# better62/MM-VQA-Healthcare

Measured on AMD Instinct MI355X. Metric: image-question pairs/sec, M3AE-base fine-tune step (fwd+bwd+AdamW) @384px, higher is better.
Workload: dtype bf16

## Files before the change

### include/m3ae_hip.h

```cpp
#ifndef M3AE_HIP_H
#define M3AE_HIP_H

#include <stdint.h>

#ifdef __cplusplus
extern "C" {
#endif

#define M3AE_ABI_VERSION 4

enum { M3AE_F32 = 0, M3AE_BF16 = 1 };
enum { M3AE_ACT_NONE = 0, M3AE_ACT_GELU = 1, M3AE_ACT_QUICKGELU = 2, M3AE_ACT_TANH = 3, M3AE_ACT_RELU = 4,
       M3AE_ACT_MULAUX = 5  };
enum { M3AE_ERR_ARG = -1, M3AE_ERR_UNSUPPORTED = -2, M3AE_ERR_ALIGN = -3, M3AE_ERR_WORKSPACE = -4 };

int m3ae_abi_version(void);
void m3ae_desc_sizes(int64_t out3[3]);
const char* m3ae_last_gemm_path(void);

typedef struct {
    int64_t M, N, K;
    int64_t batch1, batch2;
    const void* A; int64_t a_sm, a_sk, a_sb1, a_sb2;
    const void* B; int64_t b_sk, b_sn, b_sb1, b_sb2;
    void* C;       int64_t c_sm, c_sn, c_sb1, c_sb2;
    int32_t dtype_a, dtype_b, dtype_c;
    float alpha;
    int32_t accumulate;
    const float* bias;
    int32_t act;
    void* preact;
    const void* residual;
    const void* dact_aux;
    int32_t dact;
    int32_t force_generic;
    float* a_rowsum;
    float dropout_p;
    uint64_t dropout_seed;
    int32_t preact_grad;
    int32_t launch_flags;
    const void* dropout_salt;
} m3ae_gemm_desc;
enum { M3AE_GEMM_NO_PERSISTENT = 1,
       M3AE_GEMM_F32_X3 = 2,
       M3AE_GEMM_DETERMINISTIC = 4,
       M3AE_GEMM_B_TILED = 8    };
#define M3AE_GEMM_NT_VARIANT(v) ((((v) + 1) & 0xf) << 8)
#define M3AE_GEMM_TN_VARIANT(v) ((((v) + 1) & 0xf) << 12)
#define M3AE_GEMM_COL_GROUP(g) (((g) & 0xf) << 16)
int m3ae_gemm(const m3ae_gemm_desc* d, void* stream);
int m3ae_gemm_rows(const m3ae_gemm_desc* d, int64_t row_base, int64_t row_step, void* stream);
int64_t m3ae_gemm_det_workspace_bytes(const m3ae_gemm_desc* d);
int m3ae_gemm_det(const m3ae_gemm_desc* d, void* workspace, int64_t workspace_bytes, void* stream);

typedef struct {
    int64_t B, H, Lq, Lk, Dh;
    const void* q; int64_t q_sb, q_sl;
    const void* k; int64_t k_sb, k_sl;
    const void* v; int64_t v_sb, v_sl;
    void* o;       int64_t o_sb, o_sl;
    const float* key_mask;
    const float* pos_bias;
    float scale;
    int32_t causal;
    float* lse; int64_t lse_stride;
    int32_t dtype;
    void* workspace; int64_t workspace_bytes;
    const void* d_o;
    void* dq; void* dk; void* dv;
    float* delta;
    float* d_pos_bias;
    float dropout_p;
    uint64_t dropout_seed;
    const void* dropout_salt;
    int32_t launch_flags;
} m3ae_attn_desc;
enum { M3AE_ATTN_LEGACY_KERNELS = 1,
       M3AE_ATTN_F32_X3 = 2    };
int64_t m3ae_attn_workspace_bytes(const m3ae_attn_desc* d, int backward);
int m3ae_attn_fwd(const m3ae_attn_desc* d, void* stream);
int m3ae_attn_bwd(const m3ae_attn_desc* d, void* stream);
int m3ae_attn_fwd_rows(const m3ae_attn_desc* d, int64_t row_base, int64_t row_step, void* stream);
int m3ae_attn_bwd_rows(const m3ae_attn_desc* d, int64_t row_base, int64_t row_step, void* stream);
int m3ae_attn_probs(const m3ae_attn_desc* d, float* probs, int64_t p_sb, int64_t p_sh, int64_t p_sq, void* stream);
#define M3AE_ATTN_COLMEAN_F32_CHUNK 4
int64_t m3ae_attn_colmean_workspace_bytes(const m3ae_attn_desc* d);
// ... 205 lines not shown
```

### mm-vqa-healthcare_amd/csrc/gemm_mfma.hip

```cpp
#include "gemm_nt_common.h"
#include "pp_ring.h"
#include "launch.h"
#include <stdlib.h>

namespace {

constexpr int BM = 128, BN = 128, BK = 64;
constexpr int STAGE_BYTES = (BM + BN) * BK * 2;
constexpr int LDS_BYTES = 2 * STAGE_BYTES;

using namespace m3g;

template <int BM_, int BN_, int BKT, int NST, int WM, int EPI>
__global__ __launch_bounds__((BM_ / WM) * (BN_ / 64) * 64, 2) void gemm_nt_bf16_kernel(MfmaArgs a) {
    if (a.has_drop) drop_resolve(a.drop);
    constexpr int WAVES_N = BN_ / 64, NWAVES = (BM_ / WM) * WAVES_N, MI = WM / 16;
    constexpr int A_BYTES = BM_ * BKT * 2, ST_BYTES = (BM_ + BN_) * BKT * 2;
    constexpr int A_SEGS = A_BYTES / 1024 / NWAVES, B_SEGS = BN_ * BKT * 2 / 1024 / NWAVES;
    constexpr int G = A_SEGS + B_SEGS;
    extern __shared__ __attribute__((aligned(16))) char smem[];
    const int tid = threadIdx.x;
    const int lane = tid & 63;
    const int wave = __builtin_amdgcn_readfirstlane(tid >> 6);
    const int wr = wave / WAVES_N, wc = wave % WAVES_N;
// ... 554 lines not shown
        float* P = (float*)a.C + ((int64_t)split * tiles + tile_id) * (256 * 256) + ((int64_t)wave * 8 * 4 * 64 + lane) * 4;
#pragma unroll
        for (int i = 0; i < 8; ++i)
#pragma unroll
            for (int j = 0; j < 4; ++j) *(f32x4*)(P + (i * 4 + j) * 256) = acc[i][j];
        return;
    }
    if (do_rowsum && (lane & 15) == 0) {
#pragma unroll
        for (int i = 0; i < 8; ++i)
#pragma unroll
            for (int r = 0; r < 4; ++r) atomicAdd(a.a_rowsum + m0 + wr * 128 + i * 16 + 4 * (lane >> 4) + r, rsum[i][r]);
    }
    float* C = (float*)a.C;
    const bool atomic = a.splits > 1;
#pragma unroll
    for (int i = 0; i < 8; ++i)
#pragma unroll
        for (int j = 0; j < 4; ++j)
#pragma unroll
            for (int r = 0; r < 4; ++r) {
                const int64_t n1 = m0 + wr * 128 + i * 16 + 4 * (lane >> 4) + r;
                const int64_t n2 = n0 + wc * 64 + j * 16 + (lane & 15);
                float* p = C + n1 * a.ldc + n2;
                const float x = acc[i][j][r] * a.alpha;
#ifdef M3AE_EXP_TN_NOATOMIC
                asm volatile("" ::"v"(x), "v"(p));
#else
                if (atomic) atomicAdd(p, x);
                else if (a.accumulate) *p += x;
                else *p = x;
#endif
            }
}

__global__ __launch_bounds__(256) void tn_det_fold_kernel(const float* __restrict__ part, const float* __restrict__ rs_part,
                                                          float* __restrict__ C, float* __restrict__ rowsum, int64_t ldc,
                                                          int64_t M, int64_t N, int splits, int bm, int wm, float alpha,
                                                          int accumulate) {
    const int64_t plane = M * N, quads = plane / 4;
    const int waves_n = bm / 64, mi = wm / 16;
    const int64_t tile_quads = (int64_t)bm * bm / 4, tiles_n = N / bm;
    const int64_t stride = (int64_t)gridDim.x * blockDim.x;
    for (int64_t e = (int64_t)blockIdx.x * blockDim.x + threadIdx.x; e < quads; e += stride) {
        f32x4 v = *(const f32x4*)(part + e * 4);
#pragma unroll 4
        for (int sp = 1; sp < splits; ++sp) {
            const f32x4 p = *(const f32x4*)(part + sp * plane + e * 4);
            v[0] += p[0]; v[1] += p[1]; v[2] += p[2]; v[3] += p[3];
        }
        const int64_t tile = e / tile_quads;
        const int w = (int)(e - tile * tile_quads);
        const int lane = w & 63, j = (w >> 6) & 3, i = (w >> 8) % mi, wave = (w >> 8) / mi;
        const int64_t n1 = (tile / tiles_n) * bm + (wave / waves_n) * wm + i * 16 + 4 * (lane >> 4);
        const int64_t n2 = (tile % tiles_n) * bm + (wave % waves_n) * 64 + j * 16 + (lane & 15);
#pragma unroll
        for (int r = 0; r < 4; ++r) {
            float* p = C + (n1 + r) * ldc + n2;
            *p = accumulate ? *p + v[r] * alpha : v[r] * alpha;
        }
    }
    if (rowsum) {
        for (int64_t m = (int64_t)blockIdx.x * blockDim.x + threadIdx.x; m < M; m += stride) {
            float t = rs_part[m];
            for (int sp = 1; sp < splits; ++sp) t += rs_part[sp * M + m];
            rowsum[m] += t;
// ... 147 lines not shown
        g_last_path = "f32x3";
        return m3ae_gemm_f32x3(d, s, rows);
    case ROUTE_NT:
        return launch_nt(d, s, rows);
    case ROUTE_TN:
        g_last_path = "mfma_tn";
        return launch_tn(d, s);
    default:
        g_last_path = "generic";
        return m3ae_gemm_generic(d, s, rows);
    }
}

extern "C" int64_t m3ae_gemm_det_workspace_bytes(const m3ae_gemm_desc* dp) {
    if (!dp) return M3AE_ERR_ARG;
    const m3ae_gemm_desc& d = *dp;
    if (gemm_route(d) != ROUTE_TN) return 0;
    int64_t k_chunk = 0;
    const int k = tn_kernel_choice(d);
    const int64_t splits = k == 5 ? tn_pp_splits(d, &k_chunk) : tn_t_splits(d, tn_t_lds(2, k == 2 ? 32 : 64), &k_chunk);
    return tn_det_bytes(d, splits);
}

extern "C" int m3ae_gemm_det(const m3ae_gemm_desc* dp, void* workspace, int64_t workspace_bytes, void* stream) {
    if (!dp || !dp->A || !dp->B || !dp->C) return M3AE_ERR_ARG;
    const m3ae_gemm_desc& d = *dp;
    if (!(d.launch_flags & M3AE_GEMM_DETERMINISTIC)) return M3AE_ERR_ARG;
    if (d.launch_flags & M3AE_GEMM_B_TILED) return M3AE_ERR_UNSUPPORTED;
    if (gemm_route(d) != ROUTE_TN) return M3AE_ERR_UNSUPPORTED;
    if (!workspace || !aligned16(workspace) || workspace_bytes < m3ae_gemm_det_workspace_bytes(dp)) return M3AE_ERR_WORKSPACE;
    g_last_path = "mfma_tn";
    return launch_tn(d, (hipStream_t)stream, (float*)workspace);
}
```

### mm-vqa-healthcare_amd/m3ae_amd/_lib.py

```python
import ctypes as C
import os

_PKG = os.path.dirname(os.path.abspath(__file__))
DIAGNOSTIC = os.environ.get("M3AE_DIAGNOSTIC_LIB", "") == "1"
LIB_PATH = os.path.join(_PKG, "lib_diag" if DIAGNOSTIC else "lib", "libm3ae_hip.so")

F32, BF16 = 0, 1
ACT_NONE, ACT_GELU, ACT_QUICKGELU, ACT_TANH, ACT_RELU, ACT_MULAUX = 0, 1, 2, 3, 4, 5

vp, i64, i32, f32 = C.c_void_p, C.c_int64, C.c_int32, C.c_float


class GemmDesc(C.Structure):
    _fields_ = [
        ("M", i64), ("N", i64), ("K", i64), ("batch1", i64), ("batch2", i64),
        ("A", vp), ("a_sm", i64), ("a_sk", i64), ("a_sb1", i64), ("a_sb2", i64),
        ("B", vp), ("b_sk", i64), ("b_sn", i64), ("b_sb1", i64), ("b_sb2", i64),
        ("C", vp), ("c_sm", i64), ("c_sn", i64), ("c_sb1", i64), ("c_sb2", i64),
        ("dtype_a", i32), ("dtype_b", i32), ("dtype_c", i32),
        ("alpha", f32), ("accumulate", i32), ("bias", vp), ("act", i32), ("preact", vp), ("residual", vp),
        ("dact_aux", vp), ("dact", i32), ("force_generic", i32), ("a_rowsum", vp),
        ("dropout_p", f32), ("dropout_seed", C.c_uint64), ("preact_grad", i32), ("launch_flags", i32), ("dropout_salt", vp),
    ]

# ... 96 lines not shown
    "m3ae_image_resample_u8": (C.c_int, [vp, i64, vp, vp, i64, i64, i64, vp, i64, vp, vp, C.POINTER(C.c_float), C.POINTER(C.c_float), vp]),
    "m3ae_image_resample_tables": (C.c_int, [vp, i64, i64, vp, i64, vp]),
    "m3ae_image_randaug_workspace_bytes": (i64, [i64]),
    "m3ae_image_randaug_u8": (C.c_int, [vp, vp, i64, vp, i64, vp, i64, C.c_int, vp]),
    "m3ae_gemm_rows": (C.c_int, [C.POINTER(GemmDesc), i64, i64, vp]),
    "m3ae_attn_fwd_rows": (C.c_int, [C.POINTER(AttnDesc), i64, i64, vp]),
    "m3ae_attn_bwd_rows": (C.c_int, [C.POINTER(AttnDesc), i64, i64, vp]),
    "m3ae_layernorm_bwd_drop_rows": (C.c_int, [vp, vp, vp, vp, vp, vp, vp, vp, f32, C.c_uint64, vp, vp, vp, vp, i64, i64, C.c_int, i64, i64, vp]),
    "m3ae_dropout_rows": (C.c_int, [vp, vp, vp, i64, i64, f32, C.c_uint64, vp, C.c_int, i64, i64, vp]),
    "m3ae_beam_topk_workspace_bytes": (i64, [i64, i64, i64, i64]),
    "m3ae_beam_topk": (C.c_int, [vp, i64, vp, i64, i64, i64, i64, vp, i64, vp, vp, vp]),
    "m3ae_beam_step": (C.c_int, [vp, vp, vp, vp, vp, vp, vp, vp, vp, vp, vp, vp, vp, vp, i64, i64, i64, i64, i64, i64, i64, C.c_double, vp]),
    "m3ae_beam_finalize": (C.c_int, [vp, vp, vp, vp, vp, vp, vp, vp, vp, i64, i64, i64, i64, i64, i64, C.c_double, vp]),
    "m3ae_greedy_workspace_bytes": (i64, [i64, i64, i64]),
    "m3ae_greedy_argmax": (C.c_int, [vp, i64, i64, i64, i64, C.c_int, vp, i64, vp, vp]),
    "m3ae_greedy_step": (C.c_int, [vp, i64, vp, vp, vp, vp, vp, vp, i64, i64, i64, i64, i64, i64, i64, vp]),
    "m3ae_expand_samples": (C.c_int, [vp, vp, vp, i64, i64, i64, C.c_int, vp]),
    "m3ae_segment_sum_rows": (C.c_int, [vp, vp, vp, vp, i64, i64, i64, C.c_int, vp]),
    "m3ae_sumsq_workspace_bytes": (i64, [i64]),
    "m3ae_sumsq_segments": (C.c_int, [vp, i64, vp, i64, vp, i64, vp, vp, i64, vp]),
    "m3ae_clip_finalize": (C.c_int, [vp, i64, f32, f32, vp, vp]),
    "m3ae_adamw_clip": (C.c_int, [vp, vp, vp, vp, vp, i64, f32, f32, f32, f32, f32, i64, f32, vp, vp, vp]),
    "m3ae_adam": (C.c_int, [vp, vp, vp, vp, vp, i64, f32, C.c_double, C.c_double, f32, f32, i64, f32, vp]),
    "m3ae_adam_clip": (C.c_int, [vp, vp, vp, vp, vp, i64, f32, C.c_double, C.c_double, f32, f32, i64, f32, vp, vp]),
    "m3ae_sgd": (C.c_int, [vp, vp, vp, vp, i64, f32, f32, f32, f32, vp]),
    "m3ae_sgd_clip": (C.c_int, [vp, vp, vp, vp, i64, f32, f32, f32, f32, vp, vp]),
    "m3ae_layernorm_fwd_mixed": (C.c_int, [vp, vp, vp, vp, vp, vp, i64, i64, f32, vp]),
    "m3ae_layernorm_bwd_mixed": (C.c_int, [vp, vp, vp, vp, vp, vp, vp, vp, vp, vp, vp, i64, i64, vp]),
    "m3ae_layernorm_bwd_mixed_det": (C.c_int, [vp, vp, vp, vp, vp, vp, vp, vp, vp, vp, vp, i64, i64, vp]),
    "m3ae_attn_colmean_workspace_bytes": (i64, [C.POINTER(AttnDesc)]),
    "m3ae_attn_colmean": (C.c_int, [C.POINTER(AttnDesc), vp, i64, vp, i64, vp]),
    "m3ae_xattn_probs_colmean": (C.c_int, [C.POINTER(XattnDesc), C.c_int, vp, i64, vp]),
    "m3ae_heatmap_upsample": (C.c_int, [vp, i64, i64, vp, i64, i64, vp]),
}

EXPORTS = tuple(_SIGS)
_lib = None


class M3AEHipError(RuntimeError):
    pass


def lib():
    global _lib
    if _lib is None:
        if not os.path.exists(LIB_PATH):
            raise M3AEHipError(f"{LIB_PATH} is missing: build it with `python -m m3ae_amd.build` "
                               f"(or __graft_entry__.build()); this package has no CPU fallback")
        import torch
        if DIAGNOSTIC:
            import warnings
            warnings.warn(f"m3ae_amd: loading the DIAGNOSTIC library {LIB_PATH} (timing-only builds may compute wrong results)")
        l = C.CDLL(LIB_PATH)
        for name, (res, args) in _SIGS.items():
            fn = getattr(l, name)
            fn.restype, fn.argtypes = res, args
        if l.m3ae_abi_version() != ABI_VERSION:
            raise M3AEHipError(f"ABI version mismatch: library {l.m3ae_abi_version()}, binding {ABI_VERSION}")
        sizes = (i64 * 3)()
        l.m3ae_desc_sizes(sizes)
        mine = (C.sizeof(GemmDesc), C.sizeof(AttnDesc), C.sizeof(XattnDesc))
        if tuple(sizes) != mine:
            raise M3AEHipError(f"descriptor layout mismatch: library {tuple(sizes)}, binding {mine}")
        _lib = l
    return _lib
# ... 8 lines not shown
```

### mm-vqa-healthcare_amd/m3ae_amd/build.py

```python
import concurrent.futures as cf
import os
import subprocess
import sys

PKG = os.path.dirname(os.path.abspath(__file__))
ROOT = os.path.dirname(os.path.dirname(PKG))
CSRC = os.path.join(os.path.dirname(PKG), "csrc")
INC = os.path.join(ROOT, "include")
EXTRA = os.environ.get("M3AE_EXTRA_HIPCC_FLAGS", "").split()
OUT_DIR = os.path.join(PKG, "lib_diag" if EXTRA else "lib")
LIB = os.path.join(OUT_DIR, "libm3ae_hip.so")
STAMP = os.path.join(OUT_DIR, ".build_flags")
HIPCC = os.environ.get("HIPCC", "/opt/rocm/bin/hipcc")
FLAGS = ["--offload-arch=gfx950", "-O3", "-std=c++17", "-fPIC", "-Wno-unused-result", "-Wno-unused-value",
         f"-I{INC}", f"-I{CSRC}"] + EXTRA


ASM_LOAD_SOURCES = {"gemm_nt_pp2.hip": r"gemm_nt_pp2_kernel", "gemm_mfma.hip": r"gemm_nt_(bf16|pp)_kernel"}
REMARK = "-Rpass-analysis=kernel-resource-usage"


def check_no_scratch(src_name, hipcc_output):
    import re
    pat = re.compile(ASM_LOAD_SOURCES[src_name])
    name, seen, bad = None, 0, []
    for line in hipcc_output.splitlines():
        m = re.search(r"remark: Function Name: (\S+)", line)
        if m:
            name = m.group(1)
            continue
        m = re.search(r"remark:\s+ScratchSize \[bytes/lane\]: (\d+)", line)
        if m and name and pat.search(name):
            seen += 1
            if int(m.group(1)) and not re.search(r"Li5E(L[bi][0-9]E)?E+v", name):
                bad.append((name, int(m.group(1))))
    if not seen:
        raise RuntimeError(f"{src_name}: no kernel-resource-usage remarks for {ASM_LOAD_SOURCES[src_name]} (hipcc output format changed?)")
    if bad:
        raise RuntimeError(f"{src_name}: kernels with inline-asm epilogue loads use scratch memory (a spill between an asm load and "
                           f"its wait would save an in-flight register): {bad}")
    return seen


def _stale(target, deps):
    if not os.path.exists(target):
        return True
    t = os.path.getmtime(target)
    return any(os.path.getmtime(d) > t for d in deps)


def build(force=False, verbose=True):
# ... 49 lines not shown
```

### mm-vqa-healthcare_amd/m3ae_amd/ops.py

```python
import contextlib
import ctypes as C
import functools
import math
import os
import threading
from typing import NamedTuple

import torch

from . import _lib
from ._lib import (ACT_GELU, ACT_MULAUX, ACT_NONE, ACT_QUICKGELU, ACT_RELU, ACT_TANH, BF16, F32, AttnDesc, GemmDesc, XattnDesc,
                   check)

grad_ready_hook = None
SAVE_DACT = os.environ.get("M3AE_SAVE_DACT", "1") != "0"
NT_NO_PERSISTENT = os.environ.get("M3AE_NT_NO_PERSISTENT", "0") == "1"
GEMM_NT_VARIANT, GEMM_TN_VARIANT, GEMM_COL_GROUP = int(os.environ.get("M3AE_GEMM_NT_VARIANT", -1)), int(os.environ.get("M3AE_GEMM_TN_VARIANT", -1)), int(os.environ.get("M3AE_GEMM_COL_GROUP", 0))


ATTN_LEGACY = os.environ.get("M3AE_ATTN_LEGACY", "0") == "1"
GEMM_ST_POLICY = int(os.environ.get("M3AE_GEMM_ST_POLICY", 0))
TILED_B = os.environ.get("M3AE_TILED_B", "1") != "0"


# ... 274 lines not shown
         dact_aux=dact_aux, dact=dact, force_generic=force_generic, alpha=alpha, dropout=dropout,
         preact_grad=preact_grad and want_preact, rows=rows, b_tiled=tb is not None)
    return y, pre


def mm_dgrad(dy, w_param, dact_aux=None, dact=ACT_NONE, residual=None, alpha=1.0, dropout=None, out=None, ld_out=None, rows=None,
             sl=None):
    M, N = dy.shape
    wt = getattr(w_param, "m3ae_t", None)
    wtt = getattr(w_param, "m3ae_tt", None) if TILED_B and sl is None and wt is not None and dy.dtype == torch.bfloat16 else None
    if wtt is not None:
        b, b_sk, b_sn, K = wtt, 1, N, wt.shape[0]
    elif wt is not None:
        b, b_sk, b_sn, K = (wt if sl is None else wt[:, sl]), 1, wt.stride(0), wt.shape[0]
    else:
        b = compute_weight(w_param) if sl is None else compute_weight(w_param)[sl]
        b_sk, b_sn, K = b.stride(0), 1, b.shape[1]
    if out is None:
        out, ld_out = torch.empty((M, K), dtype=dy.dtype, device=dy.device), K
    gemm(dy, dy.stride(0), 1, b, b_sk, b_sn, out, ld_out, M, K, N, dact_aux=dact_aux, dact=dact, residual=residual,
         alpha=alpha, dropout=dropout, rows=rows, b_tiled=wtt is not None)
    return out


def mm_wgrad(dy, x2, ldx, w_param, b_param=None, alpha=1.0, sl=None):
    want_b = b_param is not None and b_param.requires_grad
    gb = None if not want_b else _grad_buf(b_param) if sl is None else _grad_buf(b_param)[sl]
    if not w_param.requires_grad:
        if want_b:
            colsum(dy, gb, True)
    else:
        g = _grad_buf(w_param) if sl is None else _grad_buf(w_param)[sl]
        M, N = dy.shape
        gemm(dy, 1, dy.stride(0), x2, ldx, 1, g, g.stride(0), N, g.shape[1], M, accumulate=True, alpha=alpha, a_rowsum=gb)
    if sl is None:
        if w_param.requires_grad:
            _done(w_param)
        if want_b:
            _done(b_param)


def colsum(x, out, accumulate):
    M, N = x.shape
    if _DETERMINISTIC:
        ws, n = _small_ws(_lib.DET_COLSUM, M, N, x.device)
        check(_lib.lib().m3ae_colsum_det(_p(x), _p(out), M, N, x.stride(0), _dt(x), int(accumulate), _p(ws), n, _stream()),
              "m3ae_colsum_det")
        return
    check(_lib.lib().m3ae_colsum(_p(x), _p(out), M, N, x.stride(0), _dt(x), int(accumulate), _stream()), "m3ae_colsum")


def act_bwd(dy, pre, act):
    dx = torch.empty_like(dy)
    check(_lib.lib().m3ae_act_bwd(_p(dy), _p(pre), _p(dx), dy.numel(), act, _dt(dy), _stream()), "m3ae_act_bwd")
    return dx


def _members(p):
    return getattr(p, "members", None) or ([p] if p is not None else [])


def _done(p):
    if grad_ready_hook is not None and p is not None:
        for m in _members(p):
            grad_ready_hook(m)


def _grad_buf(p):
    if getattr(p, "members", None) is not None:
        g = p.grad
        if g is None:
            raise _lib.M3AEHipError("packed parameters need ParamStore-managed gradients")
# ... 653 lines not shown
    attn_backward(*_qkv_views(proj, B), o, lse, dctx.view(o.shape), *_qkv_views(dproj, B), P.heads, mask, pos_bias, scale,
                  causal, d_pos_bias, dropout, rows)
    D = xq.shape[1]
    if len(proj) == 1:
        mm_wgrad(dproj[0], xq, D, P.w_qkv, P.b_qkv)
        return (mm_dgrad(dproj[0], P.w_qkv, residual=residual) if need_dx else None), None
    assert xkv is not None, "the forward was given ready-made kv (inference only): there is no source to differentiate"
    pq, pkv = _attn_proj(P, live=rows is not None)
    dq, dkv = dproj
    mm_wgrad(dq, xq, D, pq.w, pq.b, sl=pq.sl)
    mm_wgrad(dkv, xkv, xkv.shape[1], pkv.w, pkv.b, sl=pkv.sl)
    if pq.sl is not None:
        for prm in {id(p): p for p in (pq.w, pq.b, pkv.w, pkv.b) if p is not None}.values():
            if prm.requires_grad:
                _done(prm)
    if pq.w is pkv.w:
        dx = mm_dgrad(dkv, pkv.w, sl=pkv.sl)
        dqkv0 = torch.cat([dq, dkv.view(B, -1, dkv.shape[1])[:, 0]], dim=1)
        dx.view(B, -1, D)[:, 0] = mm_dgrad(dqkv0, pq.w, residual=residual)
        return dx, None
    dx = mm_dgrad(dq, pq.w, residual=residual, sl=pq.sl) if need_dx else None
    return dx, (mm_dgrad(dkv, pkv.w, sl=pkv.sl) if need_dsrc else None)


def _ffn_core_fwd(x2, P, act, residual, mid_drop=None, out_drop=None, rows=None):
    M, D = x2.shape
    g, u = mm_nt(x2, D, M, compute_weight(P.w1), bias=_bdata(P.b1), act=act, want_preact=True, preact_grad=SAVE_DACT,
                 dropout=mid_drop, rows=rows)
    y, _ = mm_nt(g, g.shape[1], M, compute_weight(P.w2), bias=_bdata(P.b2), residual=residual, dropout=out_drop, rows=rows,
                 out_dtype=None if residual is None else residual.dtype)
    return y, u, g


def _ffn_core_bwd(dy, x2, u, g, P, act, mid_drop=None, residual=None, rows=None):
    mm_wgrad(dy, g, g.shape[1], P.w2, P.b2)
    du = mm_dgrad(dy, P.w2, dact_aux=u, dact=ACT_MULAUX if SAVE_DACT else act, dropout=mid_drop, rows=rows)
    mm_wgrad(du, x2, x2.shape[1], P.w1, P.b1)
    return mm_dgrad(du, P.w1, residual=residual)


def _attn_sub_fwd(h2, B, L, other2, Lo, mask, P, pdrop=0.0, fused_cross=False, need_bwd=True, want_probs=False, live=False):
    if other2 is not None and fused_cross and not live and xattn_supported(h2, L, other2, Lo, mask, P, backward=need_bwd):
        return xattn_fwd(h2, B, L, other2, Lo, mask, P, pdrop, need_bwd=need_bwd, want_probs=want_probs)
    da, dh = dropout_pair(pdrop), dropout_pair(pdrop)
    rows = (0, L) if live else None
    xkv = h2 if other2 is None else other2
    o, lse, proj = _attn_core_fwd(h2, xkv, B, P, mask=mask, dropout=da, rows=rows)
    M, n = h2.shape[0], o.shape[2]
    s, _ = mm_nt(o.view(M, n), n, M, compute_weight(P.w_o), bias=_bdata(P.b_o), residual=h2, dropout=dh, rows=rows)
    y, mean, rstd = ln_fwd_raw(s, P.ln)
    return y, (h2, xkv, proj, o, lse, s, mean, rstd, mask, da, dh, rows)


def _attn_sub_probs(saved, B, L, Lo, P):
    if isinstance(saved[0], str):
        return xattn_probs(saved)
    q3, k3, _ = _qkv_views(saved[2], B)
    lse, mask, da = saved[4], saved[8], saved[9]
    return attn_probs(q3, k3, lse, P.heads, mask, dropout=da)


def _attn_sub_colmean(saved, B, L, Lo, P):
    if isinstance(saved[0], str):
        return xattn_colmean(saved)
    q3, k3, _ = _qkv_views(saved[2], B)
    lse, mask, da = saved[4], saved[8], saved[9]
    return attn_colmean(q3, k3, lse, P.heads, mask, dropout=da)


def _post_ln_bwd(dy, s, ln, mean, rstd, dh, rows=None):
    if dh is not None:
        return ln_bwd_raw(dy, s, ln, mean, rstd, drop=dh, rows=rows)
    ds = ln_bwd_raw(dy, s, ln, mean, rstd)
    return ds, ds


def _attn_sub_bwd(dy, saved, B, L, Lo, P, need_dother=True):
    if isinstance(saved[0], str):
        return xattn_bwd(dy, saved, B, L, Lo, P, need_dother)
    h2, xkv, proj, o, lse, s, mean, rstd, mask, da, dh, rows = saved
    M, n = h2.shape[0], o.shape[2]
    ds, dsd = _post_ln_bwd(dy, s, P.ln, mean, rstd, dh, rows)
    mm_wgrad(dsd, o.view(M, n), n, P.w_o, P.b_o)
    dctx = mm_dgrad(dsd, P.w_o)
    return _attn_core_bwd(dctx, h2, xkv, proj, o, lse, B, P, mask=mask, dropout=da, residual=ds, need_dsrc=need_dother, rows=rows)


def _ffn_sub_fwd(h2, P, pdrop=0.0, rows=None):
    dh = dropout_pair(pdrop)
    s, u, g = _ffn_core_fwd(h2, P, ACT_GELU, h2, out_drop=dh, rows=rows)
    y, mean, rstd = ln_fwd_raw(s, P.ln)
    return y, (h2, u, g, s, mean, rstd, dh, rows)


def _ffn_sub_bwd(dy, saved, P):
    h2, u, g, s, mean, rstd, dh, rows = saved
    ds, dsd = _post_ln_bwd(dy, s, P.ln, mean, rstd, dh, rows)
    return _ffn_core_bwd(dsd, h2, u, g, P, ACT_GELU, residual=ds, rows=rows)


class BlockOpts(NamedTuple):
    pdrop: float = 0.0
    cls_only: bool = False
    fused_cross: bool = False
    want_probs: bool = False
    need_bwd: bool = True
    want_summary: bool = False


# ... 1 lines not shown

    @staticmethod
    def forward(ctx, h, other, mask_self, mask_other, P, opts, *anchors):
        B, L, D = h.shape
        Lo = other.shape[1]
        h2 = h.contiguous().view(B * L, D)
        other2 = other.contiguous().view(B * Lo, other.shape[2])
        pd, live = opts.pdrop, opts.cls_only
        q2, kv2 = (h2.view(B, L, D)[:, 0].contiguous(), h2) if live else (h2, None)
        a, s1 = _attn_sub_fwd(q2, B, L, kv2, L, mask_self, P.attn, pd, live=live)
        c, s2 = _attn_sub_fwd(a, B, L, other2, Lo, mask_other, P.cross, pd, fused_cross=opts.fused_cross, need_bwd=opts.need_bwd,
                              want_probs=opts.want_probs or opts.want_summary, live=live)
        y, s3 = _ffn_sub_fwd(c, P.ffn, pd, rows=(0, L) if live else None)
        ctx.saved = (s1, s2, s3)
        ctx.P, ctx.dims, ctx.n_anchor = P, (B, L, Lo, D), len(anchors)
        ctx.need_other = other.requires_grad
        extra = ()
        if opts.want_probs:
            extra += (_attn_sub_probs(s1, B, L, L, P.attn), _attn_sub_probs(s2, B, L, Lo, P.cross))
        if opts.want_summary:
            assert not live, "attention summaries are full-layer outputs"
            extra += (_attn_sub_colmean(s1, B, L, L, P.attn), _attn_sub_colmean(s2, B, L, Lo, P.cross))
        if extra:
            ctx.mark_non_differentiable(*extra)
            return (y.view(B, L, D),) + extra
        return y.view(B, -1, D)

    @staticmethod
    def backward(ctx, dy, *_maps):
        B, L, Lo, D = ctx.dims
        s1, s2, s3 = ctx.saved
        ctx.saved = None
        P = ctx.P
        dc = _ffn_sub_bwd(dy.contiguous().view(-1, D), s3, P.ffn)
        da, dother = _attn_sub_bwd(dc, s2, B, L, Lo, P.cross, need_dother=ctx.need_other)
        dh, _ = _attn_sub_bwd(da, s1, B, L, L, P.attn)
        return (dh.view(B, L, D), None if dother is None else dother.view(B, Lo, -1), None, None, None, None) + \
               (None,) * ctx.n_anchor


class BertSelfLayerFn(Function):

    @staticmethod
    def forward(ctx, h, mask, P, opts, *anchors):
        B, L, D = h.shape
        h2 = h.contiguous().view(B * L, D)
        a, s1 = _attn_sub_fwd(h2, B, L, None, L, mask, P.attn, opts.pdrop)
        y, s3 = _ffn_sub_fwd(a, P.ffn, opts.pdrop)
        ctx.saved = (s1, s3)
        ctx.P, ctx.dims, ctx.n_anchor = P, (B, L, D), len(anchors)
        return y.view(B, L, D)

    @staticmethod
    def backward(ctx, dy):
        B, L, D = ctx.dims
        s1, s3 = ctx.saved
        ctx.saved = None
        da = _ffn_sub_bwd(dy.contiguous().view(B * L, D), s3, ctx.P.ffn)
        dh, _ = _attn_sub_bwd(da, s1, B, L, L, ctx.P.attn)
        return (dh.view(B, L, D), None, None, None) + (None,) * ctx.n_anchor


class ClipBlockFn(Function):

    @staticmethod
    def forward(ctx, x, P, *anchors):
        B, L, D = x.shape
        M = B * L
        x2 = x.contiguous().view(M, D)
        lo = compute_weight(P.w_qkv).dtype
        h1, m1, r1 = ln_fwd_raw(x2, P.ln1, out_dtype=lo)
        o, lse, proj = _attn_core_fwd(h1, h1, B, P)
        xa, _ = mm_nt(o.view(M, D), D, M, compute_weight(P.w_o), bias=_bdata(P.b_o), residual=x2, out_dtype=x2.dtype)
        h2, m2, r2 = ln_fwd_raw(xa, P.ln2, out_dtype=lo)
        y, u, g = _ffn_core_fwd(h2, P, ACT_QUICKGELU, xa)
        ctx.saved = (x2, m1, r1, h1, proj, o, lse, xa, m2, r2, h2, u, g)
        ctx.P, ctx.dims, ctx.n_anchor = P, (B, L, D), len(anchors)
        return y.view(B, L, D)

    @staticmethod
    def backward(ctx, dy):
        B, L, D = ctx.dims
        M = B * L
        x2, m1, r1, h1, proj, o, lse, xa, m2, r2, h2, u, g = ctx.saved
        ctx.saved = None
        P = ctx.P
        dy2 = dy.contiguous().view(M, D)
        mixed = h2.dtype != xa.dtype
        dh2 = _ffn_core_bwd(cast(dy2, h2.dtype), h2, u, g, P, ACT_QUICKGELU)
        if mixed:
            dxa_s, dxa = ln_bwd_raw(dh2, xa, P.ln2, m2, r2, dx_add=dy2, want_lo=True)
        else:
            dxa_s = dxa = ln_bwd_raw(dh2, xa, P.ln2, m2, r2, dx_add=dy2)
        mm_wgrad(dxa, o.view(M, D), D, P.w_o, P.b_o)
        dctx = mm_dgrad(dxa, P.w_o)
        dh1, _ = _attn_core_bwd(dctx, h1, h1, proj, o, lse, B, P)
        dx = ln_bwd_raw(dh1, x2, P.ln1, m1, r1, dx_add=dxa_s)
        return (dx.view(B, L, D), None) + (None,) * ctx.n_anchor


def _drop_raw(x2, drop):
    if drop is None:
        return x2
    x2 = x2.contiguous()
    out = torch.empty_like(x2)
    check(_lib.lib().m3ae_dropout(_p(x2), _p(out), None, x2.shape[0], x2.shape[1], drop[0], drop[1], _salt(), _dt(x2), _stream()),
          "m3ae_dropout")
    return out


def t5_attn_fwd(h2, B, P, bias, causal, pdrop=0.0, src2=None, kv=None):
    da, dh = dropout_pair(pdrop), dropout_pair(pdrop)
    n, _, rstd = ln_fwd_raw(h2, P.ln, rms=True)
    xkv = n if (src2 is None and kv is None) else src2
    o, lse, proj = _attn_core_fwd(n, xkv, B, P, kv=kv, pos_bias=bias, scale=1.0, causal=causal, dropout=da)
    M, inner = h2.shape[0], o.shape[2]
    y, _ = mm_nt(o.view(M, inner), inner, M, compute_weight(P.w_o), residual=h2, dropout=dh)
    return y, (h2, rstd, n, proj, o, lse, xkv, da, dh)


def t5_self_attn_step(h2, B, P, bias_row, cache, t, pdrop=0.0):
    da, dh = dropout_pair(pdrop), dropout_pair(pdrop)
    n, _, _ = ln_fwd_raw(h2, P.ln, rms=True)
    D = n.shape[1]
    inner = P.w_o.shape[1]
    qkv, _ = mm_nt(n, D, B, compute_weight(P.w_qkv))
    cache[:, t].copy_(qkv[:, inner:])
    q = qkv[:, :inner].unsqueeze(1)
    o, _ = attn_forward(q, cache[:, :t + 1, :inner], cache[:, :t + 1, inner:], P.heads, None, bias_row, scale=1.0,
                        causal=False, dropout=da)
# ... 678 lines not shown
```

Baseline: 1447.

## Batch per-layer weight-gradient GEMMs into one grouped persistent TN kernel

Adds a grouped TN GEMM kernel that runs up to eight weight-gradient GEMMs in one launch. Each workgroup walks its units across members and prefetches the next member's first chunks while it writes back the current tile. On the Python side, wgrad calls inside each layer's backward are deferred into a thread-local queue and flushed at scope exit; gradient-ready callbacks fire only at flush time. The aim is to cut launch overhead and tail underutilisation of small wgrad GEMMs. The cost is that wgrad is delayed to the end of the layer scope, which may reduce overlap with gradient reduction and keeps activations alive longer.

```diff
diff --git a/include/m3ae_hip.h b/include/m3ae_hip.h
--- a/include/m3ae_hip.h
+++ b/include/m3ae_hip.h
@@ -52,6 +52,7 @@
 int m3ae_gemm_rows(const m3ae_gemm_desc* d, int64_t row_base, int64_t row_step, void* stream);
 int64_t m3ae_gemm_det_workspace_bytes(const m3ae_gemm_desc* d);
 int m3ae_gemm_det(const m3ae_gemm_desc* d, void* workspace, int64_t workspace_bytes, void* stream);
+int m3ae_gemm_wgrad_group(const m3ae_gemm_desc* descs, int n, void* stream);
 
 typedef struct {
     int64_t B, H, Lq, Lk, Dh;
diff --git a/mm-vqa-healthcare_amd/csrc/gemm_mfma.hip b/mm-vqa-healthcare_amd/csrc/gemm_mfma.hip
--- a/mm-vqa-healthcare_amd/csrc/gemm_mfma.hip
+++ b/mm-vqa-healthcare_amd/csrc/gemm_mfma.hip
@@ -610,6 +610,190 @@
                 else *p = x;
 #endif
             }
+}
+
+constexpr int TN_GROUP_MAX = 8;
+struct TnGroupMember {
+    const bf16_t* A; int64_t lda;
+    const bf16_t* B; int64_t ldb;
+    float* C; int64_t ldc;
+    float* a_rowsum;
+    int64_t K, k_chunk;
+    unsigned tiles_n, tiles, units;
+    int splits, accumulate;
+    float alpha;
+};
+struct TnGroupArgs {
+    TnGroupMember m[TN_GROUP_MAX];
+    int n;
+};
+struct TnUnit {
+    const bf16_t* A; int64_t lda;
+    const bf16_t* B; int64_t ldb;
+    int64_t m0, n0, r_begin, r_end;
+    int nc;
+};
+DEVINL TnUnit tn_group_unit(const TnGroupMember& g, unsigned bid) {
+    const unsigned wg = xcd_remap(bid, g.units);
+    const unsigned tile_id = wg % g.tiles, split = wg / g.tiles;
+    TnUnit u;
+    u.A = g.A; u.lda = g.lda; u.B = g.B; u.ldb = g.ldb;
+    u.m0 = (int64_t)(tile_id / g.tiles_n) * 256;
+    u.n0 = (int64_t)(tile_id % g.tiles_n) * 256;
+    u.r_begin = (int64_t)split * g.k_chunk;
+    u.r_end = u.r_begin + g.k_chunk < g.K ? u.r_begin + g.k_chunk : g.K;
+    u.nc = (int)((u.r_end - u.r_begin + 31) / 32);
+    return u;
+}
+
+__global__ __launch_bounds__(512, 2) void gemm_tn_pp_group_kernel(TnGroupArgs g) {
+    constexpr int CK = 32, NW = 8, A_BYTES = 256 * CK * 2, SLOT = 2 * A_BYTES;
+    constexpr int DEPTH = 3, G = 4;
+    extern __shared__ __attribute__((aligned(16))) char smem[];
+    const int tid = threadIdx.x;
+    const int lane = tid & 63;
+    const int wave = __builtin_amdgcn_readfirstlane(tid >> 6);
+    const int wr = wave >> 2, wc = wave & 3;
+    const s16x8 ones = {0x3F80, 0x3F80, 0x3F80, 0x3F80, 0x3F80, 0x3F80, 0x3F80, 0x3F80};
+
+    int mi = 0;
+    TnUnit u = tn_group_unit(g.m[0], blockIdx.x);
+#pragma unroll
+    for (int c = 0; c < 3; ++c) {
+        if (c < u.nc) {
+            const int64_t r0 = u.r_begin + (int64_t)c * CK;
+            tn_stage<256, 2, NW>(u.B, u.ldb, r0, u.r_end, u.n0, smem + c * SLOT + A_BYTES, wave, lane);
+            tn_stage<256, 2, NW>(u.A, u.lda, r0, u.r_end, u.m0, smem + c * SLOT, wave, lane);
+        }
+    }
+    bool carried = false;
+    for (;;) {
+        const int nc = u.nc;
+        f32x4 acc[8][4];
+#pragma unroll
+        for (int i = 0; i < 8; ++i)
+#pragma unroll
+            for (int j = 0; j < 4; ++j) acc[i][j] = (f32x4){0.f, 0.f, 0.f, 0.f};
+        const bool do_rowsum = g.m[mi].a_rowsum != nullptr && u.n0 == 0 && wc == 0;
+        f32x4 rsum[8];
+#pragma unroll
+        for (int i = 0; i < 8; ++i) rsum[i] = (f32x4){0.f, 0.f, 0.f, 0.f};
+
+        if (carried) wait_vm<63>();
+        else wait_vm_chunks<G, DEPTH - 1>(pp_inflight_prologue<DEPTH>(nc));
+        PP_FENCE();
+        __builtin_amdgcn_s_barrier();
+        PP_FENCE();
+        if (wr == 1) { __builtin_amdgcn_s_barrier(); PP_FENCE(); }
+
+        for (int c = 0; c < nc; ++c) {
+            const char* At = smem + (c & 3) * SLOT;
+            const char* Bt = At + A_BYTES;
+            char* nxt = smem + ((c + 3) & 3) * SLOT;
+            const bool more = c + 3 < nc;
+            const int64_t r3 = u.r_begin + (int64_t)(c + 3) * CK;
+            s16x8 bfr[4], af[4];
+#pragma unroll
+            for (int j = 0; j < 4; ++j) bfr[j] = tn_frag<256>(Bt, 0, wc * 64 + j * 16, lane);
+#pragma unroll
+            for (int i = 0; i < 4; ++i) af[i] = tn_frag<256>(At, 0, wr * 128 + i * 16, lane);
+            if (more) tn_stage<256, 2, NW>(u.B, u.ldb, r3, u.r_end, u.n0, nxt + A_BYTES, wave, lane);
+            PP_FENCE();
+            __builtin_amdgcn_s_barrier();
+            PP_FENCE();
+            asm volatile("s_waitcnt lgkmcnt(0)" ::: "memory");
+            __builtin_amdgcn_sched_barrier(0);
+            __builtin_amdgcn_s_setprio(1);
+#pragma unroll
+            for (int i = 0; i < 4; ++i) {
+#pragma unroll
+                for (int j = 0; j < 4; ++j)
+                    acc[i][j] = __builtin_amdgcn_mfma_f32_16x16x32_bf16(
+                        __builtin_bit_cast(bf16x8_t, af[i]), __builtin_bit_cast(bf16x8_t, bfr[j]), acc[i][j], 0, 0, 0);
+            }
+            if (do_rowsum) {
+#pragma unroll
+                for (int i = 0; i < 4; ++i)
+                    rsum[i] = __builtin_amdgcn_mfma_f32_16x16x32_bf16(
+                        __builtin_bit_cast(bf16x8_t, af[i]), __builtin_bit_cast(bf16x8_t, ones), rsum[i], 0, 0, 0);
+            }
+            __builtin_amdgcn_s_setprio(0);
+            PP_FENCE();
+            __builtin_amdgcn_s_barrier();
+            PP_FENCE();
+#pragma unroll
+            for (int i = 0; i < 4; ++i) af[i] = tn_frag<256>(At, 0, wr * 128 + 64 + i * 16, lane);
+            if (more) tn_stage<256, 2, NW>(u.A, u.lda, r3, u.r_end, u.m0, nxt, wave, lane);
+            wait_vm_chunks<G, DEPTH - 1>(pp_inflight_next<DEPTH>(nc, c));
+            PP_FENCE();
+            __builtin_amdgcn_s_barrier();
+            PP_FENCE();
+            asm volatile("s_waitcnt lgkmcnt(0)" ::: "memory");
+            __builtin_amdgcn_sched_barrier(0);
+            __builtin_amdgcn_s_setprio(1);
+#pragma unroll
+            for (int i = 0; i < 4; ++i) {
+#pragma unroll
+                for (int j = 0; j < 4; ++j)
+                    acc[4 + i][j] = __builtin_amdgcn_mfma_f32_16x16x32_bf16(
+                        __builtin_bit_cast(bf16x8_t, af[i]), __builtin_bit_cast(bf16x8_t, bfr[j]), acc[4 + i][j], 0, 0, 0);
+            }
+            if (do_rowsum) {
+#pragma unroll
+                for (int i = 0; i < 4; ++i)
+                    rsum[4 + i] = __builtin_amdgcn_mfma_f32_16x16x32_bf16(
+                        __builtin_bit_cast(bf16x8_t, af[i]), __builtin_bit_cast(bf16x8_t, ones), rsum[4 + i], 0, 0, 0);
+            }
+            __builtin_amdgcn_s_setprio(0);
+            PP_FENCE();
+            __builtin_amdgcn_s_barrier();
+            PP_FENCE();
+        }
+        if (wr == 0) { __builtin_amdgcn_s_barrier(); PP_FENCE(); }
+
+        const int nmi = mi + 1;
+        const bool has_next = nmi < g.n && blockIdx.x < g.m[nmi].units;
+        const int64_t m0 = u.m0, n0 = u.n0;
+        if (has_next) {
+            u = tn_group_unit(g.m[nmi], blockIdx.x);
+#pragma unroll
+            for (int c = 0; c < 3; ++c) {
+                if (c < u.nc) {
+                    const int64_t r0 = u.r_begin + (int64_t)c * CK;
+                    tn_stage<256, 2, NW>(u.B, u.ldb, r0, u.r_end, u.n0, smem + c * SLOT + A_BYTES, wave, lane);
+                    tn_stage<256, 2, NW>(u.A, u.lda, r0, u.r_end, u.m0, smem + c * SLOT, wave, lane);
+                }
+            }
+            PP_FENCE();
+        }
+
+        const TnGroupMember& me = g.m[mi];
+        if (do_rowsum && (lane & 15) == 0) {
+#pragma unroll
+            for (int i = 0; i < 8; ++i)
+#pragma unroll
+                for (int r = 0; r < 4; ++r) atomicAdd(me.a_rowsum + m0 + wr * 128 + i * 16 + 4 * (lane >> 4) + r, rsum[i][r]);
+        }
+        float* C = me.C;
+        const int64_t ldc = me.ldc;
+        const float alpha = me.alpha;
+        const int form = me.splits > 1 ? 0 : me.accumulate ? 1 : 2;
+        float* C0 = C + (m0 + wr * 128 + 4 * (lane >> 4)) * ldc + n0 + wc * 64 + (lane & 15);
+        auto walk = [&](auto&& put) {
+#pragma unroll
+            for (int i = 0; i < 8; ++i)
+#pragma unroll
+                for (int j = 0; j < 4; ++j)
+#pragma unroll
+                    for (int r = 0; r < 4; ++r) put(C0 + (i * 16 + r) * ldc + j * 16, acc[i][j][r] * alpha);
+        };
+        if (form == 0) walk([](float* p, float x) { atomicAdd(p, x); });
+        else if (form == 1) walk([](float* p, float x) { *p += x; });
+        else walk([](float* p, float x) { *p = x; });
+        if (!has_next) return;
+        mi = nmi;
+        carried = true;
+    }
 }
 
 __global__ __launch_bounds__(256) void tn_det_fold_kernel(const float* __restrict__ part, const float* __restrict__ rs_part,
@@ -823,3 +1007,37 @@
     g_last_path = "mfma_tn";
     return launch_tn(d, (hipStream_t)stream, (float*)workspace);
 }
+
+extern "C" int m3ae_gemm_wgrad_group(const m3ae_gemm_desc* descs, int n, void* stream) {
+    if (!descs || n < 1 || n > TN_GROUP_MAX) return M3AE_ERR_ARG;
+    TnGroupArgs g{};
+    g.n = n;
+    for (int i = 0; i < n; ++i) {
+        const m3ae_gemm_desc& d = descs[i];
+        if (!d.A || !d.B || !d.C) return M3AE_ERR_ARG;
+        const GemmRoute route = gemm_route(d);
+        if (route == ROUTE_BAD_DIMS) return M3AE_ERR_ARG;
+        if (route != ROUTE_TN || (d.launch_flags & (M3AE_GEMM_DETERMINISTIC | M3AE_GEMM_B_TILED)) || d.M % 256 != 0 || d.N % 256 != 0)
+            return M3AE_ERR_UNSUPPORTED;
+        TnGroupMember m{};
+        m.A = (const bf16_t*)d.A; m.lda = d.a_sk;
+        m.B = (const bf16_t*)d.B; m.ldb = d.b_sk;
+        m.C = (float*)d.C; m.ldc = d.c_sm;
+        m.a_rowsum = d.a_rowsum;
+        m.K = d.K;
+        m.splits = (int)tn_pp_splits(d, &m.k_chunk);
+        if (m.k_chunk < 8 * 32) return M3AE_ERR_UNSUPPORTED;
+        m.tiles_n = (unsigned)(d.N / 256);
+        m.tiles = (unsigned)(d.M / 256) * m.tiles_n;
+        if ((int64_t)m.tiles * m.splits > 65535) return M3AE_ERR_UNSUPPORTED;
+        m.units = m.tiles * (unsigned)m.splits;
+        m.accumulate = d.accumulate;
+        m.alpha = d.alpha;
+        int at = i;
+        while (at > 0 && g.m[at - 1].units < m.units) { g.m[at] = g.m[at - 1]; --at; }
+        g.m[at] = m;
+    }
+    constexpr int lds = 4 * (256 + 256) * 32 * 2;
+    g_last_path = "mfma_tn_group";
+    return launch_dyn<gemm_tn_pp_group_kernel>(dim3(g.m[0].units), dim3(512), lds, (hipStream_t)stream, g);
+}
diff --git a/mm-vqa-healthcare_amd/m3ae_amd/_lib.py b/mm-vqa-healthcare_amd/m3ae_amd/_lib.py
--- a/mm-vqa-healthcare_amd/m3ae_amd/_lib.py
+++ b/mm-vqa-healthcare_amd/m3ae_amd/_lib.py
@@ -152,6 +152,7 @@
     "m3ae_attn_colmean": (C.c_int, [C.POINTER(AttnDesc), vp, i64, vp, i64, vp]),
     "m3ae_xattn_probs_colmean": (C.c_int, [C.POINTER(XattnDesc), C.c_int, vp, i64, vp]),
     "m3ae_heatmap_upsample": (C.c_int, [vp, i64, i64, vp, i64, i64, vp]),
+    "m3ae_gemm_wgrad_group": (C.c_int, [C.POINTER(GemmDesc), C.c_int, vp]),
 }
 
 EXPORTS = tuple(_SIGS)
diff --git a/mm-vqa-healthcare_amd/m3ae_amd/build.py b/mm-vqa-healthcare_amd/m3ae_amd/build.py
--- a/mm-vqa-healthcare_amd/m3ae_amd/build.py
+++ b/mm-vqa-healthcare_amd/m3ae_amd/build.py
@@ -16,7 +16,7 @@
          f"-I{INC}", f"-I{CSRC}"] + EXTRA
 
 
-ASM_LOAD_SOURCES = {"gemm_nt_pp2.hip": r"gemm_nt_pp2_kernel", "gemm_mfma.hip": r"gemm_nt_(bf16|pp)_kernel"}
+ASM_LOAD_SOURCES = {"gemm_nt_pp2.hip": r"gemm_nt_pp2_kernel", "gemm_mfma.hip": r"gemm_nt_(bf16|pp)_kernel|gemm_tn_pp_group_kernel"}
 REMARK = "-Rpass-analysis=kernel-resource-usage"
 
 
diff --git a/mm-vqa-healthcare_amd/m3ae_amd/ops.py b/mm-vqa-healthcare_amd/m3ae_amd/ops.py
--- a/mm-vqa-healthcare_amd/m3ae_amd/ops.py
+++ b/mm-vqa-healthcare_amd/m3ae_amd/ops.py
@@ -330,12 +330,82 @@
     else:
         g = _grad_buf(w_param) if sl is None else _grad_buf(w_param)[sl]
         M, N = dy.shape
+        q = _WGQ.members
+        if (q is not None and sl is None and M >= WGRAD_GROUP_MIN_ROWS and not _DETERMINISTIC and not NT_NO_PERSISTENT
+                and dy.dtype == torch.bfloat16 and x2.dtype == torch.bfloat16):
+            q.append((dy, x2, ldx, g, gb, alpha, w_param, b_param if want_b else None))
+            return
         gemm(dy, 1, dy.stride(0), x2, ldx, 1, g, g.stride(0), N, g.shape[1], M, accumulate=True, alpha=alpha, a_rowsum=gb)
     if sl is None:
         if w_param.requires_grad:
             _done(w_param)
         if want_b:
             _done(b_param)
+
+
+WGRAD_GROUP = os.environ.get("M3AE_WGRAD_GROUP", "1") != "0"
+WGRAD_GROUP_MIN_ROWS = 16384
+WGRAD_GROUP_MAX = 8
+_ERR_UNSUPPORTED = -2
+
+
+class _WgradQueue(threading.local):
+    members = None
+
+
+_WGQ = _WgradQueue()
+
+
+def _wgrad_desc(dy, x2, ldx, g, gb, alpha):
+    d = GemmDesc()
+    d.M, d.N, d.K = dy.shape[1], g.shape[1], dy.shape[0]
+    d.batch1, d.batch2 = 1, 1
+    d.A, d.a_sm, d.a_sk = dy.data_ptr(), 1, dy.stride(0)
+    d.B, d.b_sk, d.b_sn = x2.data_ptr(), ldx, 1
+    d.C, d.c_sm, d.c_sn = g.data_ptr(), g.stride(0), 1
+    d.dtype_a, d.dtype_b, d.dtype_c = BF16, BF16, F32
+    d.alpha, d.accumulate = alpha, 1
+    d.launch_flags = _gemm_flags()
+    if gb is not None:
+        d.a_rowsum = gb.data_ptr()
+    return d
+
+
+def _wgrad_flush(members):
+    lib = _lib.lib()
+    for i in range(0, len(members), WGRAD_GROUP_MAX):
+        part = members[i:i + WGRAD_GROUP_MAX]
+        rc = _ERR_UNSUPPORTED
+        if len(part) > 1:
+            descs = (GemmDesc * len(part))(*[_wgrad_desc(*m[:6]) for m in part])
+            e0 = _prof_begin()
+            rc = lib.m3ae_gemm_wgrad_group(descs, len(part), _stream())
+            if rc == 0 and e0 is not None:
+                ks = {m[0].shape[0] for m in part}
+                mn = sum(m[0].shape[1] * m[3].shape[1] * (1 if len(ks) == 1 else m[0].shape[0]) for m in part)
+                _prof_end(e0, "gemm:mfma_tn_group", (mn, 1, ks.pop() if len(ks) == 1 else 1, 1))
+        if rc == _ERR_UNSUPPORTED:
+            for dy, x2, ldx, g, gb, alpha, _, _ in part:
+                gemm(dy, 1, dy.stride(0), x2, ldx, 1, g, g.stride(0), dy.shape[1], g.shape[1], dy.shape[0], accumulate=True,
+                     alpha=alpha, a_rowsum=gb)
+        else:
+            check(rc, "m3ae_gemm_wgrad_group")
+    for m in members:
+        _done(m[6])
+        _done(m[7])
+
+
+@contextlib.contextmanager
+def wgrad_group():
+    if not WGRAD_GROUP or _WGQ.members is not None:
+        yield
+        return
+    _WGQ.members = members = []
+    try:
+        yield
+    finally:
+        _WGQ.members = None
+    _wgrad_flush(members)
 
 
 def colsum(x, out, accumulate):
@@ -1055,6 +1125,7 @@
     return y, u, g
 
 
+@wgrad_group()
 def _ffn_core_bwd(dy, x2, u, g, P, act, mid_drop=None, residual=None, rows=None):
     mm_wgrad(dy, g, g.shape[1], P.w2, P.b2)
     du = mm_dgrad(dy, P.w2, dact_aux=u, dact=ACT_MULAUX if SAVE_DACT else act, dropout=mid_drop, rows=rows)
@@ -1098,6 +1169,7 @@
     return ds, ds
 
 
+@wgrad_group()
 def _attn_sub_bwd(dy, saved, B, L, Lo, P, need_dother=True):
     if isinstance(saved[0], str):
         return xattn_bwd(dy, saved, B, L, Lo, P, need_dother)
@@ -1165,9 +1237,10 @@
         s1, s2, s3 = ctx.saved
         ctx.saved = None
         P = ctx.P
-        dc = _ffn_sub_bwd(dy.contiguous().view(-1, D), s3, P.ffn)
-        da, dother = _attn_sub_bwd(dc, s2, B, L, Lo, P.cross, need_dother=ctx.need_other)
-        dh, _ = _attn_sub_bwd(da, s1, B, L, L, P.attn)
+        with wgrad_group():
+            dc = _ffn_sub_bwd(dy.contiguous().view(-1, D), s3, P.ffn)
+            da, dother = _attn_sub_bwd(dc, s2, B, L, Lo, P.cross, need_dother=ctx.need_other)
+            dh, _ = _attn_sub_bwd(da, s1, B, L, L, P.attn)
         return (dh.view(B, L, D), None if dother is None else dother.view(B, Lo, -1), None, None, None, None) + \
                (None,) * ctx.n_anchor
 
@@ -1189,8 +1262,9 @@
         B, L, D = ctx.dims
         s1, s3 = ctx.saved
         ctx.saved = None
-        da = _ffn_sub_bwd(dy.contiguous().view(B * L, D), s3, ctx.P.ffn)
-        dh, _ = _attn_sub_bwd(da, s1, B, L, L, ctx.P.attn)
+        with wgrad_group():
+            da = _ffn_sub_bwd(dy.contiguous().view(B * L, D), s3, ctx.P.ffn)
+            dh, _ = _attn_sub_bwd(da, s1, B, L, L, ctx.P.attn)
         return (dh.view(B, L, D), None, None, None) + (None,) * ctx.n_anchor
 
 
@@ -1220,15 +1294,16 @@
         P = ctx.P
         dy2 = dy.contiguous().view(M, D)
         mixed = h2.dtype != xa.dtype
-        dh2 = _ffn_core_bwd(cast(dy2, h2.dtype), h2, u, g, P, ACT_QUICKGELU)
-        if mixed:
-            dxa_s, dxa = ln_bwd_raw(dh2, xa, P.ln2, m2, r2, dx_add=dy2, want_lo=True)
-        else:
-            dxa_s = dxa = ln_bwd_raw(dh2, xa, P.ln2, m2, r2, dx_add=dy2)
-        mm_wgrad(dxa, o.view(M, D), D, P.w_o, P.b_o)
-        dctx = mm_dgrad(dxa, P.w_o)
-        dh1, _ = _attn_core_bwd(dctx, h1, h1, proj, o, lse, B, P)
-        dx = ln_bwd_raw(dh1, x2, P.ln1, m1, r1, dx_add=dxa_s)
+        with wgrad_group():
+            dh2 = _ffn_core_bwd(cast(dy2, h2.dtype), h2, u, g, P, ACT_QUICKGELU)
+            if mixed:
+                dxa_s, dxa = ln_bwd_raw(dh2, xa, P.ln2, m2, r2, dx_add=dy2, want_lo=True)
+            else:
+                dxa_s = dxa = ln_bwd_raw(dh2, xa, P.ln2, m2, r2, dx_add=dy2)
+            mm_wgrad(dxa, o.view(M, D), D, P.w_o, P.b_o)
+            dctx = mm_dgrad(dxa, P.w_o)
+            dh1, _ = _attn_core_bwd(dctx, h1, h1, proj, o, lse, B, P)
+            dx = ln_bwd_raw(dh1, x2, P.ln1, m1, r1, dx_add=dxa_s)
         return (dx.view(B, L, D), None) + (None,) * ctx.n_anchor
 
 
```

Result: no change. 1458, median of 2 (+0.8%).
